# vimalabs/VIMA

Hardware: NVIDIA H100
Metric: policy steps/sec (batched action decode) (higher is better)
Workload: dtype f16 hi*hi + e4m3 cross terms (2 tensor pass-equivalents), f16 3-term in attention, fp32 accumulate/softmax/LN

## Files before the change

### vima_b200/build.py

```python
from __future__ import annotations

import hashlib
import os
import subprocess
import sys
from concurrent.futures import ThreadPoolExecutor

HERE = os.path.dirname(os.path.abspath(__file__))
CSRC = os.path.join(HERE, "csrc")
OUT_DIR = os.path.join(HERE, "_lib")
LIB_PATH = os.path.join(OUT_DIR, "libvima_b200.so")
SOURCES = ["api.cu", "gemm_tc_f16.cu", "gemm_tc_f16x3.cu", "gemm_tc_f16f8.cu", "gemm_tc_bf16.cu", "gemm_tc_bf16x3.cu", "gemm_wide_f16f8.cu", "norm.cu", "attention.cu", "attention_tc.cu", "attention_tc_paged.cu", "attention_tail.cu", "gemm_simt.cu", "misc.cu", "prepare.cu", "slots.cu"]
HEADERS = ["common.cuh", "kernels.h", "attention_tc.cuh", "gemm_tc.cuh", "gemm_tc_variants.cuh", "gemm_wide.cuh", os.path.join("..", "..", "include", "vima_b200.h")]
NVCC_FLAGS = [
    "-gencode", "arch=compute_90a,code=sm_90a", "-O3", "-lineinfo", "-std=c++17", "--expt-relaxed-constexpr",
    "-Xcompiler", "-fPIC", "-Xcompiler", "-fvisibility=hidden",
]


def _nvcc() -> str:
    for p in (os.environ.get("NVCC"), "/usr/local/cuda/bin/nvcc", "nvcc"):
        if p and (os.path.isfile(p) or p == "nvcc"):
            return p
    raise RuntimeError("nvcc not found")


def _digest() -> str:
    h = hashlib.sha256()
    for f in SOURCES + HEADERS:
        with open(os.path.join(CSRC, f), "rb") as fh:
            h.update(fh.read())
    h.update(" ".join(NVCC_FLAGS).encode())
    return h.hexdigest()


# ... 34 lines not shown
```

### vima_b200/csrc/api.cu

```cuda
#include <cstdarg>
#include <cstddef>
#include <cstdio>
#include <cstring>
#include <cstdlib>

#include "../../include/vima_b200.h"
#include "gemm_wide.cuh"
#include "kernels.h"

using namespace vima;
static_assert(VIMA_KV_PAGE_TOKENS == KV_PAGE_TOKENS, "page size of the C ABI and of the kernels");

struct vima_ctx {
  int device;
  int sm_count;
  int max_smem_optin;
  long long launches;
  char err[512];
  void* encode_tiled;
  int attn_tc;
  int attn_tail;
  int epi_prefetch;
  int attn_bias_tc;
  int gemm_wide;
};

struct DeviceGuard {
  int prev = -1;
  bool armed = false;
  cudaError_t enter(int dev) {
    cudaError_t e = cudaGetDevice(&prev);
    if (e != cudaSuccess) return e;
    if (prev == dev) return cudaSuccess;
    armed = true;
    return cudaSetDevice(dev);
  }
  ~DeviceGuard() {
    if (armed) cudaSetDevice(prev);
  }
};

static int fail(vima_ctx* c, int code, const char* fmt, ...) {
  if (c) {
    va_list ap;
    va_start(ap, fmt);
    vsnprintf(c->err, sizeof(c->err), fmt, ap);
    va_end(ap);
// ... 30 lines not shown
    return VIMA_OK;                                      \
  }

extern "C" {

int vima_abi_version(void) { return VIMA_B200_ABI_VERSION; }

int vima_set_option(vima_ctx* c, const char* key, const char* value) {
  if (!c) return VIMA_E_INVALID;
  if (!key || !value) return fail(c, VIMA_E_INVALID, "set_option: null key or value");
  if (!strcmp(key, "attn")) {
    if (!strcmp(value, "tc")) { c->attn_tc = 1; return VIMA_OK; }
    if (!strcmp(value, "mma")) { c->attn_tc = 0; return VIMA_OK; }
  } else if (!strcmp(key, "attn_tail")) {
    if (!strcmp(value, "kernel")) { c->attn_tail = 1; return VIMA_OK; }
    if (!strcmp(value, "off")) { c->attn_tail = 0; return VIMA_OK; }
  } else if (!strcmp(key, "attn_bias")) {
    if (!strcmp(value, "auto")) { c->attn_bias_tc = 0; return VIMA_OK; }
    if (!strcmp(value, "tc")) { c->attn_bias_tc = 1; return VIMA_OK; }
  } else if (!strcmp(key, "epi_prefetch")) {
    if (!strcmp(value, "0") || !strcmp(value, "1")) { c->epi_prefetch = value[0] == '1'; return VIMA_OK; }
  } else if (!strcmp(key, "gemm_wide")) {
    if (!strcmp(value, "0") || !strcmp(value, "1")) { c->gemm_wide = value[0] == '1'; return VIMA_OK; }
  }
  return fail(c, VIMA_E_INVALID, "set_option: unknown option %s=%s", key, value);
}

int vima_create(vima_ctx** out, int device) {
  if (!out) return VIMA_E_INVALID;
  *out = nullptr;
  int n = 0;
  if (cudaGetDeviceCount(&n) != cudaSuccess || device < 0 || device >= n) return VIMA_E_CUDA;
  cudaDeviceProp prop;
  if (cudaGetDeviceProperties(&prop, device) != cudaSuccess) return VIMA_E_CUDA;
  if (prop.major != 9 || prop.minor != 0) return VIMA_E_UNSUPPORTED;
  vima_ctx* c = new vima_ctx();
  memset(c, 0, sizeof(*c));
  c->device = device;
  c->sm_count = prop.multiProcessorCount;
  c->max_smem_optin = (int)prop.sharedMemPerBlockOptin;
  DeviceGuard guard;
  if (guard.enter(device) != cudaSuccess) { delete c; return VIMA_E_CUDA; }
  cudaFree(0);
  cudaDriverEntryPointQueryResult q;
  void* fn = nullptr;
  if (cudaGetDriverEntryPoint("cuTensorMapEncodeTiled", &fn, cudaEnableDefault, &q) != cudaSuccess || fn == nullptr) {
    delete c;
    return VIMA_E_CUDA;
  }
  c->encode_tiled = fn;
  c->attn_tc = 1; c->attn_tail = 1; c->epi_prefetch = 0; c->attn_bias_tc = 0; c->gemm_wide = 1;
  if (const char* e = getenv("VIMA_B200_ATTN")) vima_set_option(c, "attn", e);
  if (const char* e = getenv("VIMA_B200_ATTN_TAIL")) vima_set_option(c, "attn_tail", e);
  if (const char* e = getenv("VIMA_B200_EPI_PREFETCH")) vima_set_option(c, "epi_prefetch", e);
  if (const char* e = getenv("VIMA_B200_ATTN_BIAS")) vima_set_option(c, "attn_bias", e);
  if (const char* e = getenv("VIMA_B200_GEMM_WIDE")) vima_set_option(c, "gemm_wide", e);
  c->err[0] = 0;
  *out = c;
  return VIMA_OK;
}

void vima_destroy(vima_ctx* c) { delete c; }
const char* vima_last_error(vima_ctx* c) { return c ? c->err : "null context"; }
int vima_sm_count(vima_ctx* c) { return c ? c->sm_count : 0; }
int vima_sizeof_gemm_desc(void) { return (int)sizeof(vima_gemm_desc); }
int vima_sizeof_norm_desc(void) { return (int)sizeof(vima_norm_desc); }
int vima_sizeof_attn_desc(void) { return (int)sizeof(vima_attn_desc); }
int vima_sizeof_f32_gemm_group(void) { return (int)sizeof(vima_f32_gemm_group); }
int64_t vima_launch_count(vima_ctx* c) { return c ? c->launches : 0; }

int vima_split_f32(vima_ctx* c, const float* x, int64_t rows, int cols, int ldx, void* hi, void* lo, int ld16, int pad_cols, float scale,
                   int dtype, void* stream) {
  CHECK_CTX(c);
  if (!x || !hi || pad_cols < cols || pad_cols > ld16) return fail(c, VIMA_E_INVALID, "split_f32: bad arguments");
  LAUNCHED(c, launch_split(x, rows, cols, ldx, (unsigned short*)hi, (unsigned short*)lo, ld16, pad_cols, scale, dtype, (cudaStream_t)stream),
           "split_f32");
}

int vima_pack_weight(vima_ctx* c, const float* w, int n, int k, int transposed, int ldw, void* hi, void* lo, int ld16, float scale, int dtype,
// ... 220 lines not shown
  p.key_mask = d->key_mask; p.rel_bias = d->rel_bias;
  p.o_hi = (unsigned short*)d->o_hi; p.o_lo = (unsigned short*)d->o_lo; p.ldo = d->ldo;
  p.B = d->B; p.H = d->H; p.Lq = d->Lq; p.Lk = d->Lk; p.D = d->D;
  p.scale = d->scale; p.causal = d->causal; p.split = split; p.dtype = d->dtype;
  p.o_lo8 = (unsigned char*)d->o_lo8; p.o_hi8 = (unsigned char*)d->o_hi8; p.ldo8 = d->ldo8;
  p.kv_batch_rows = d->kv_batch_rows; p.mask_ld = d->mask_ld; p.q_pos0 = d->q_pos0; p.q_batch_rows = 0;
  p.q_pos = d->q_pos;
  p.kv_pages = d->kv_pages; p.kv_page_ld = d->kv_page_ld; p.kv_pool_pages = d->kv_pool_pages;
  p.kv_len = d->kv_len;
  if (d->kv_pages && ((d->causal && !d->q_pos) || d->rel_bias || d->kv_page_ld < 1 || d->kv_pool_pages < 1 ||
                      d->Lk > (long long)d->kv_page_ld * VIMA_KV_PAGE_TOKENS || (long long)d->kv_pool_pages * VIMA_KV_PAGE_TOKENS > 0x7fffffffll))
    return fail(c, VIMA_E_INVALID, "attention: paged k / v need q_pos (or non-causal attention), no relative bias, Lk <= kv_page_ld*%d (Lk %d, "
                "kv_page_ld %d) and 1 <= kv_pool_pages with kv_pool_pages*%d rows inside the 32-bit row range (kv_pool_pages %d)",
                VIMA_KV_PAGE_TOKENS, d->Lk, d->kv_page_ld, VIMA_KV_PAGE_TOKENS, d->kv_pool_pages);
  if (d->kv_len && (d->causal || d->q_pos || d->rel_bias))
    return fail(c, VIMA_E_INVALID, "attention: per-batch kv_len needs non-causal attention without q_pos or relative bias");
  if ((d->kv_batch_rows && d->kv_batch_rows < d->Lk) || (d->mask_ld && d->mask_ld < d->Lk) || d->q_pos0 < 0)
    return fail(c, VIMA_E_INVALID, "attention: kv_batch_rows / mask_ld must cover Lk, q_pos0 >= 0");
  if (d->q_pos && (!d->causal || d->rel_bias || d->Lq > d->Lk))
    return fail(c, VIMA_E_INVALID, "attention: per-batch q_pos needs causal attention, no relative bias and Lq <= Lk");
  if ((p.o_lo8 == nullptr) != (p.o_hi8 == nullptr) || (p.o_lo8 && ((p.ldo8 & 1) || d->dtype != DT_F16)))
    return fail(c, VIMA_E_INVALID, "attention: o_lo8/o_hi8 come together (fp16 format, even ldo8)");
  if (c->attn_tc && attention_tc_supported(p)) {
    const int tail = p.Lq % 128;
    if (c->attn_tail && p.Lq > 128 && tail >= 1 && tail <= ATTN_TAIL_MAX_ROWS && p.Lk <= ATTN_TAIL_MAX_LK) {
      AttnParams body = p;
      body.Lq = p.Lq - tail;
      body.q_batch_rows = p.Lq;
      cudaError_t e_ = launch_attention_tc(body, c->encode_tiled, (cudaStream_t)stream);
      if (e_ != cudaSuccess) return cuda_fail(c, e_, "attention_tc");
      c->launches++;
      LAUNCHED(c, launch_attention_tail(p, p.Lq - tail, tail, (cudaStream_t)stream), "attention_tail");
    }
    LAUNCHED(c, launch_attention_tc(p, c->encode_tiled, (cudaStream_t)stream), "attention_tc");
  }
  if (c->attn_tc && attention_bias_tc_supported(p) && (c->attn_bias_tc || attention_smem_bytes(p) > (size_t)c->max_smem_optin))
    LAUNCHED(c, launch_attention_tc(p, c->encode_tiled, (cudaStream_t)stream), "attention_bias_tc");
  {
    const size_t need = attention_smem_bytes(p);
    if (need > (size_t)c->max_smem_optin)
      return fail(c, VIMA_E_UNSUPPORTED,
                  "attention: Lk = %d keys of head_dim %d (%s operands%s) need %zu bytes of shared memory, the device offers %d: the "
                  "resident-K/V kernel takes Lk <= %d at this head_dim", d->Lk, d->D, split ? "split" : "single", d->rel_bias ? ", relative bias" : "",
                  need, c->max_smem_optin, attention_max_lk(p, (size_t)c->max_smem_optin));
  }
  LAUNCHED(c, launch_attention(p, (cudaStream_t)stream), "attention");
}

int vima_latent_attention(vima_ctx* c, const float* q, int ldq, int64_t q_batch_stride, const float* k, int ldk, const float* v, int ldv, float* o,
                          int ldo, int64_t N, int Lq, int Lk, int H, int d, float scale, void* stream) {
  CHECK_CTX(c);
  if (!q || !k || !v || !o) return fail(c, VIMA_E_INVALID, "latent_attention: null pointer");
  if (Lk < 1 || Lk > 16 || d < 1 || d > 128 || Lq < 0 || N < 0 || H < 1)
    return fail(c, VIMA_E_UNSUPPORTED, "latent_attention: 1..16 keys, head_dim <= 128 (Lk %d, d %d)", Lk, d);
  LatentAttnParams p;
  p.q = q; p.ldq = ldq; p.q_batch_stride = q_batch_stride; p.k = k; p.ldk = ldk; p.v = v; p.ldv = ldv; p.o = o; p.ldo = ldo;
  p.N = N; p.Lq = Lq; p.Lk = Lk; p.H = H; p.d = d; p.scale = scale;
// ... 296 lines not shown
```

### vima_b200/csrc/attention_tc.cu

```cuda
#include "attention_tc.cuh"

namespace vima {

namespace {

template <int DT>
__global__ void __launch_bounds__(ATC_THREADS, 2) attention_tc_kernel(const __grid_constant__ AttnTcParams P) {
  attention_tc_body<DT, 32, true, false, false>(P);
}
template <int DT, bool SPLIT>
__global__ void __launch_bounds__(ATC_THREADS, 2) attention_bias_tc_kernel(const __grid_constant__ AttnTcParams P) {
  attention_tc_body<DT, 64, SPLIT, true, false>(P);
}

bool aligned_operands(const AttnParams& p) {
  auto al = [](const void* q) { return ((uintptr_t)q & 15) == 0; };
  return al(p.q_hi) && al(p.q_lo) && al(p.k_hi) && al(p.k_lo) && al(p.v_hi) && al(p.v_lo) && al(p.o_hi) && al(p.o_lo) && al(p.o_lo8) &&
         al(p.o_hi8);
}

}

long long attention_kv_rows(const AttnParams& p) {
  if (p.kv_pages) return (long long)p.kv_pool_pages * KV_PAGE_TOKENS;
  return (long long)p.B * (p.kv_batch_rows ? p.kv_batch_rows : p.Lk);
}

bool attention_tc_supported(const AttnParams& p) {
  const int qbr = p.q_batch_rows ? p.q_batch_rows : p.Lq;
  if (!aligned_operands(p)) return false;
  return p.D == 32 && p.split != 0 && p.rel_bias == nullptr && p.q_lo && p.k_lo && p.v_lo && (p.ldq % 8 == 0) && (p.ldk % 8 == 0) &&
         (p.ldv % 8 == 0) && (p.ldo % 8 == 0) && (p.o_lo8 == nullptr || p.ldo8 % 8 == 0) && p.H <= 65535 && p.B <= 65535 && p.Lk >= 1 &&
         attention_kv_rows(p) <= 0x7fffffffll && (long long)p.B * qbr <= 0x7fffffffll;
}

bool attention_bias_tc_supported(const AttnParams& p) {
  if (!aligned_operands(p)) return false;
  const bool split_ok = p.split ? (p.q_lo && p.k_lo && p.v_lo) : (!p.q_lo && !p.k_lo && !p.v_lo);
  return p.D == 64 && p.rel_bias != nullptr && !p.causal && p.q_pos == nullptr && p.q_pos0 == 0 && p.q_batch_rows == 0 && p.Lq == p.Lk &&
         (p.kv_batch_rows == 0 || p.kv_batch_rows == p.Lk) && (p.mask_ld == 0 || p.mask_ld == p.Lk) && split_ok && (p.ldq % 8 == 0) &&
         (p.ldk % 8 == 0) && (p.ldv % 8 == 0) && (p.ldo % 2 == 0) && (p.o_lo8 == nullptr || p.ldo8 % 2 == 0) && p.H <= 65535 &&
         p.B <= 65535 && p.Lk >= 1 && (long long)p.B * p.Lk <= 0x7fffffffll;
}

cudaError_t launch_attention_tc(const AttnParams& p, void* encode_fn, cudaStream_t stream) {
  if (p.B == 0 || p.Lq == 0) return cudaSuccess;
  const bool bias = p.rel_bias != nullptr;
  const int D = bias ? 64 : 32;
  AttnTcParams P;
  memset(&P, 0, sizeof(P));
  P.a = p;
  const long long kv_rows = attention_kv_rows(p);
  const long long q_rows = (long long)p.B * (p.q_batch_rows ? p.q_batch_rows : p.Lq);
  auto map = [&](CUtensorMap* tm, const void* base, long long rows, int ld, int box_rows) {
    return encode_tmap_2d(encode_fn, tm, p.dtype == DT_BF16 ? CU_TENSOR_MAP_DATA_TYPE_BFLOAT16 : CU_TENSOR_MAP_DATA_TYPE_FLOAT16, base,
                          (uint64_t)rows, (uint64_t)p.H * D, (uint64_t)ld * 2, (uint32_t)D, (uint32_t)box_rows,
                          D == 32 ? CU_TENSOR_MAP_SWIZZLE_64B : CU_TENSOR_MAP_SWIZZLE_128B, CU_TENSOR_MAP_L2_PROMOTION_L2_128B) == CUDA_SUCCESS;
  };
  bool ok = map(&P.tm_q_hi, p.q_hi, q_rows, p.ldq, ATC_BM) && map(&P.tm_k_hi, p.k_hi, kv_rows, p.ldk, ATC_KC);
  if (p.split) ok = ok && map(&P.tm_q_lo, p.q_lo, q_rows, p.ldq, ATC_BM) && map(&P.tm_k_lo, p.k_lo, kv_rows, p.ldk, ATC_KC);
  if (!ok) return cudaErrorInvalidValue;
  dim3 grid((p.Lq + ATC_BM - 1) / ATC_BM, p.H, p.B);
  const bool bf = p.dtype == DT_BF16;
  if (!bias && p.kv_pages) return launch_attention_tc_paged(P, grid, stream);
  if (!bias) return bf ? launch_t<attention_tc_kernel<DT_BF16>, 32, false>(P, grid, stream) : launch_t<attention_tc_kernel<DT_F16>, 32, false>(P, grid, stream);
  if (bf) return p.split ? launch_t<attention_bias_tc_kernel<DT_BF16, true>, 64, true>(P, grid, stream)
                         : launch_t<attention_bias_tc_kernel<DT_BF16, false>, 64, true>(P, grid, stream);
  return p.split ? launch_t<attention_bias_tc_kernel<DT_F16, true>, 64, true>(P, grid, stream)
                 : launch_t<attention_bias_tc_kernel<DT_F16, false>, 64, true>(P, grid, stream);
}

}
```

### vima_b200/csrc/attention_tc.cuh

```cuda
#pragma once
#include "kernels.h"

namespace vima {

struct AttnTcParams {
  AttnParams a;
  CUtensorMap tm_q_hi, tm_q_lo, tm_k_hi, tm_k_lo;
};
cudaError_t launch_attention_tc_paged(const AttnTcParams& P, dim3 grid, cudaStream_t stream);

namespace {

constexpr int ATC_THREADS = 256;
constexpr int ATC_BM = 128, ATC_KC = 64;
constexpr int ATC_WIN = ATC_BM + ATC_KC - 1;

template <int D, bool BIAS>
struct AtcSmem {
  static constexpr int Q_PART = ATC_BM * D * 2;
  static constexpr int K_PART = ATC_KC * D * 2;
  static constexpr int QH = 0, QL = Q_PART;
  static constexpr int K = 2 * Q_PART;
  static constexpr int VT = K + 4 * K_PART;
  static constexpr int MASK = VT + 4 * K_PART;
  static constexpr int BIAS_W = MASK + 2 * ATC_KC * 4;
  static constexpr int BAR = BIAS_W + (BIAS ? 2 * 192 * 4 : 0);
  static constexpr int BYTES = BAR + 32;
};

template <int DT, int D, bool SPLIT, bool BIAS, bool PAGED>
__device__ __forceinline__ void attention_tc_body(const AttnTcParams& P) {
  using S = AtcSmem<D, BIAS>;
  constexpr int PARTS = SPLIT ? 2 : 1;
  constexpr int VN = D / 4;
  const AttnParams& p = P.a;
  extern __shared__ __align__(1024) uint8_t sm[];
  float* maskadd = reinterpret_cast<float*>(sm + S::MASK);
  float* sbias = reinterpret_cast<float*>(sm + S::BIAS_W);
  uint64_t* bars = reinterpret_cast<uint64_t*>(sm + S::BAR);
  uint64_t* q_full = bars + 0;
  uint64_t* k_full = bars + 1;

  const int tid = threadIdx.x, warp = tid >> 5, lane = tid & 31;
  const int wg = warp >> 2;
  const int q0 = blockIdx.x * ATC_BM, h = blockIdx.y, b = blockIdx.z;
  const int Lq = p.Lq;
  const int mld = !BIAS && p.mask_ld ? p.mask_ld : p.Lk;
  const int qbr = !BIAS && p.q_batch_rows ? p.q_batch_rows : Lq;
  int qp0 = 0, Lk = p.Lk;
  if constexpr (!BIAS) attn_batch_keys(p, b, qbr, qp0, Lk);
  const uint32_t sbase = smem_u32(sm);
// ... 57 lines not shown
  const float c_l2 = p.scale * LOG2E;
  auto desc_qk = [](uint32_t addr) { return D == 32 ? wgmma_desc_sw64(addr) : wgmma_desc_sw128(addr); };
  const uint64_t dqh = desc_qk(sbase + S::QH + wg * (S::Q_PART / 2)), dql = desc_qk(sbase + S::QL + wg * (S::Q_PART / 2));
  const int vj = tid >> 2, vd = tid & 3;
  uint32_t k_use[2] = {0u, 0u};
  float o[D / 2], m_run[2], l_run[2];
  int n = n_plan;
  for (int pass = 0; pass < 2; ++pass) {
#pragma unroll
    for (int i = 0; i < D / 2; ++i) o[i] = 0.f;
    m_run[0] = m_run[1] = -INFINITY;
    l_run[0] = l_run[1] = 0.f;
    if (tid == 0) {
      load_k(0, 0);
      if (n > 1) load_k(1, 1);
    }
    if (pass == 0) mbar_wait(q_full, 0);
    for (int c = 0; c < n; ++c) {
      const int stage = c & 1;
      const int k0 = c * ATC_KC;
      mbar_wait(&k_full[stage], k_use[stage] & 1u);
      k_use[stage]++;
      float s[32];
      {
        const uint32_t k_addr = sbase + S::K + stage * 2 * S::K_PART;
        const uint64_t dkh = desc_qk(k_addr), dkl = desc_qk(k_addr + S::K_PART);
        wgmma_fence();
#pragma unroll
        for (int k = 0; k < D / 16; ++k) wgmma_m64nNk16_ss<DT, 64>(s, dqh + 2 * k, dkh + 2 * k, (uint32_t)(k != 0));
        if constexpr (SPLIT) {
#pragma unroll
          for (int k = 0; k < D / 16; ++k) wgmma_m64nNk16_ss<DT, 64>(s, dql + 2 * k, dkh + 2 * k, 1u);
#pragma unroll
          for (int k = 0; k < D / 16; ++k) wgmma_m64nNk16_ss<DT, 64>(s, dqh + 2 * k, dkl + 2 * k, 1u);
        }
        wgmma_commit();
      }
      {
        uint4 vh[VN / 8], vl[VN / 8];
#pragma unroll
        for (int i = 0; i < VN / 8; ++i) vh[i] = vl[i] = make_uint4(0u, 0u, 0u, 0u);
        if (k0 + vj < Lk) {
          const size_t off = (size_t)(chunk_row(c) + vj) * p.ldv + x_col + vd * VN;
#pragma unroll
          for (int i = 0; i < VN / 8; ++i) {
            vh[i] = __ldg(reinterpret_cast<const uint4*>(p.v_hi + off + 8 * i));
            if constexpr (SPLIT) vl[i] = __ldg(reinterpret_cast<const uint4*>(p.v_lo + off + 8 * i));
          }
        }
        if (c + 1 < n) stage_chunk(c + 1);
        uint8_t* vt = sm + S::VT + stage * 2 * S::K_PART;
        uint32_t wh[VN / 2], wl[VN / 2];
#pragma unroll
        for (int i = 0; i < VN / 8; ++i) {
          wh[4 * i] = vh[i].x; wh[4 * i + 1] = vh[i].y; wh[4 * i + 2] = vh[i].z; wh[4 * i + 3] = vh[i].w;
          wl[4 * i] = vl[i].x; wl[4 * i + 1] = vl[i].y; wl[4 * i + 2] = vl[i].z; wl[4 * i + 3] = vl[i].w;
        }
#pragma unroll
        for (int e = 0; e < VN; ++e) {
          const int nn = vd * VN + e;
          const int off = nn * 128 + ((((vj >> 3) ^ (nn & 7))) << 4) + (vj & 7) * 2;
          *reinterpret_cast<unsigned short*>(vt + off) = (unsigned short)(wh[e >> 1] >> (16 * (e & 1)));
          if constexpr (SPLIT) *reinterpret_cast<unsigned short*>(vt + S::K_PART + off) = (unsigned short)(wl[e >> 1] >> (16 * (e & 1)));
        }
        fence_proxy_async();
      }
      wgmma_wait<0>();
      wgmma_fence_acc(s);
      const float* mk = maskadd + stage * ATC_KC;
      const float* bw = sbias + stage * 192 + (ATC_BM - 1) - r_loc;
      float mx[2] = {-INFINITY, -INFINITY};
#pragma unroll
      for (int g = 0; g < 8; ++g)
#pragma unroll
        for (int e = 0; e < 4; ++e) {
          const int jj = 8 * g + 2 * qd + (e & 1), key = k0 + jj;
          const float mm = mk[jj];
          float y;
          if constexpr (BIAS) {
            y = s[4 * g + e] * c_l2;
            y += bw[jj - 8 * (e >> 1)];
            y += mm;
          } else {
            y = fmaf(s[4 * g + e], c_l2, mm);
            if (p.causal && key > q0 + r_loc + 8 * (e >> 1) + qp0) y = CAUSAL_L2 + mm;
          }
          s[4 * g + e] = y;
          mx[e >> 1] = fmaxf(mx[e >> 1], y);
        }
      float f[2];
#pragma unroll
      for (int hh = 0; hh < 2; ++hh) {
        mx[hh] = fmaxf(mx[hh], __shfl_xor_sync(0xffffffffu, mx[hh], 1));
        mx[hh] = fmaxf(mx[hh], __shfl_xor_sync(0xffffffffu, mx[hh], 2));
        const float m_new = fmaxf(m_run[hh], mx[hh]);
        f[hh] = ex2_approx(m_run[hh] - m_new);
        m_run[hh] = m_new;
      }
      uint32_t ph[16], pl[16];
      float ps[2] = {0.f, 0.f};
#pragma unroll
      for (int i = 0; i < 16; ++i) {
        const int hh = i & 1;
        const float p0 = ex2_approx(s[2 * i] - m_run[hh]), p1 = ex2_approx(s[2 * i + 1] - m_run[hh]);
        ps[hh] += p0 + p1;
        split2<DT>(p0, p1, ph[i], pl[i]);
      }
#pragma unroll
      for (int hh = 0; hh < 2; ++hh) l_run[hh] = l_run[hh] * f[hh] + ps[hh];
#pragma unroll
      for (int i = 0; i < D / 2; ++i) o[i] *= f[(i >> 1) & 1];
      named_bar_sync(1, ATC_THREADS);
      if (tid == 0 && c + 2 < n) load_k(c + 2, stage);
      {
        const uint32_t vt_addr = sbase + S::VT + stage * 2 * S::K_PART;
        const uint64_t dvh = wgmma_desc_sw128(vt_addr), dvl = wgmma_desc_sw128(vt_addr + S::K_PART);
        wgmma_fence();
#pragma unroll
        for (int kk = 0; kk < ATC_KC / 16; ++kk) {
          const uint32_t ah[4] = {ph[4 * kk], ph[4 * kk + 1], ph[4 * kk + 2], ph[4 * kk + 3]};
          const uint32_t al[4] = {pl[4 * kk], pl[4 * kk + 1], pl[4 * kk + 2], pl[4 * kk + 3]};
          wgmma_m64nNk16_rs<DT, D>(o, ah, dvh + 2 * kk, 1u);
          if constexpr (SPLIT) {
            wgmma_m64nNk16_rs<DT, D>(o, al, dvh + 2 * kk, 1u);
            wgmma_m64nNk16_rs<DT, D>(o, ah, dvl + 2 * kk, 1u);
          }
        }
        wgmma_commit();
        wgmma_wait<0>();
        wgmma_fence_acc(o);
      }
    }
    if (pass == 1 || !may_rerun) break;
    if constexpr (!BIAS) {
      const int undone = (r_loc < rows_here && !(m_run[0] > EXIT_L2)) || (r_loc + 8 < rows_here && !(m_run[1] > EXIT_L2));
      if (!__syncthreads_or(undone)) break;
      n = n_all;
      stage_chunk(0);
      __syncthreads();
    }
  }
#pragma unroll
  for (int hh = 0; hh < 2; ++hh) {
    float l = l_run[hh];
    l += __shfl_xor_sync(0xffffffffu, l, 1);
    l += __shfl_xor_sync(0xffffffffu, l, 2);
    const int row = q0 + r_loc + 8 * hh;
    if (row < Lq) {
      const float inv = 1.0f / l;
      const size_t brow = (size_t)b * qbr + row;
#pragma unroll
      for (int g = 0; g < D / 8; ++g) attn_store_pair<DT>(p, brow, x_col + 8 * g + 2 * qd, o[4 * g + 2 * hh] * inv, o[4 * g + 2 * hh + 1] * inv);
    }
  }
}

template <auto KERNEL, int D, bool BIAS>
cudaError_t launch_t(const AttnTcParams& P, dim3 grid, cudaStream_t stream) {
  constexpr int smem = AtcSmem<D, BIAS>::BYTES;
  const cudaError_t e = raise_smem_ceiling<KERNEL>(smem);
  if (e != cudaSuccess) return e;
  KERNEL<<<grid, ATC_THREADS, smem, stream>>>(P);
  return cudaGetLastError();
}

}

}
```

### vima_b200/csrc/kernels.h

```cpp
#pragma once
#include "common.cuh"

namespace vima {

struct NormParams {
  const float* x; long long rows; int cols; int ldx;
  const float* add; int ld_add;
  const float* w; const float* b;
  float eps; int rms;
  const float* w2; const float* b2; float eps2;
  float* out_f32; int ld_o32;
  float* out2_f32; int ld_o2;
  unsigned short* out_hi; unsigned short* out_lo; int ld_o16;
  int dtype;
  unsigned char* out_lo8; unsigned char* out_hi8; int ld_o8;
  float* stats_out; float stats_eps;
};
cudaError_t launch_norm(const NormParams& p, cudaStream_t stream);
cudaError_t launch_row_stats_finalize(const float* partial, long long rows, int parts, int cols, float eps, int rms, float* stats,
                                      cudaStream_t stream);

struct AttnParams {
  const unsigned short *q_hi, *q_lo; int ldq;
  const unsigned short *k_hi, *k_lo; int ldk;
// ... 44 lines not shown
  split2<DT>(x0, x1, hi, lo);
  const size_t off = brow * p.ldo + col;
  *reinterpret_cast<uint32_t*>(p.o_hi + off) = hi;
  if (p.o_lo) *reinterpret_cast<uint32_t*>(p.o_lo + off) = lo;
  if (p.o_lo8) {
    const float2 f = __half22float2(*reinterpret_cast<const __half2*>(&hi));
    const size_t off8 = brow * p.ldo8 + col;
    unsigned short l8, h8;
    asm("cvt.rn.satfinite.e4m3x2.f32 %0, %1, %2;" : "=h"(l8) : "f"((x1 - f.y) * F8_ACT_LO_SCALE), "f"((x0 - f.x) * F8_ACT_LO_SCALE));
    asm("cvt.rn.satfinite.e4m3x2.f32 %0, %1, %2;" : "=h"(h8) : "f"(x1 * F8_ACT_HI_SCALE), "f"(x0 * F8_ACT_HI_SCALE));
    *reinterpret_cast<unsigned short*>(p.o_lo8 + off8) = l8;
    *reinterpret_cast<unsigned short*>(p.o_hi8 + off8) = h8;
  }
}
constexpr int ATTN_TAIL_MAX_ROWS = 8;
constexpr int ATTN_TAIL_MAX_LK = 512;
cudaError_t launch_attention(const AttnParams& p, cudaStream_t stream);
size_t attention_smem_bytes(const AttnParams& p);
int attention_max_lk(const AttnParams& p, size_t smem_limit);
long long attention_kv_rows(const AttnParams& p);
bool attention_tc_supported(const AttnParams& p);
bool attention_bias_tc_supported(const AttnParams& p);
cudaError_t launch_attention_tc(const AttnParams& p, void* encode_tiled_fn, cudaStream_t stream);
cudaError_t launch_attention_tail(const AttnParams& p, int row0, int nt, cudaStream_t stream);

struct SmallAttnParams {
  const float* qkv; int ld;
  unsigned short *o_hi, *o_lo; int ldo; float* o_f32;
  long long N; int S, H, W; float scale; int dtype;
};
cudaError_t launch_small_attention(const SmallAttnParams& p, cudaStream_t stream);

struct LatentAttnParams {
  const float* q; int ldq; long long q_batch_stride;
  const float* k; int ldk;
  const float* v; int ldv;
  float* o; int ldo;
  long long N; int Lq, Lk, H, d; float scale;
};
cudaError_t launch_latent_attention(const LatentAttnParams& p, cudaStream_t stream);

struct SimtGemmGroup {
  const float* x; int ldx;
  const float* w; int ldw;
  const float* b;
  float* y; int ldy;
// ... 80 lines not shown
```

Baseline: 1633.

## Add resident-KV attention kernel that keeps all keys/values in shared memory per head

Adds an attention kernel that launches one CTA per (head, batch), loads the whole K and transposed V for short sequences (up to 320 keys) into shared memory once, then has its two warpgroups pull 64-row query blocks through a shared atomic counter with double-buffered Q loads. The target cost is the repeated K/V staging and per-chunk barriers that the tiled kernel pays for every 128-row query tile. The shared QK/softmax/PV pieces are factored into helpers that both kernels use. The new path is on by default when shapes fit, and it trades grid parallelism for reuse, so small batch×head counts may leave SMs idle.

New measurement: 1650, median of 6. +1.0%, better.

```diff
diff --git a/vima_b200/build.py b/vima_b200/build.py
--- a/vima_b200/build.py
+++ b/vima_b200/build.py
@@ -10,7 +10,7 @@
 CSRC = os.path.join(HERE, "csrc")
 OUT_DIR = os.path.join(HERE, "_lib")
 LIB_PATH = os.path.join(OUT_DIR, "libvima_b200.so")
-SOURCES = ["api.cu", "gemm_tc_f16.cu", "gemm_tc_f16x3.cu", "gemm_tc_f16f8.cu", "gemm_tc_bf16.cu", "gemm_tc_bf16x3.cu", "gemm_wide_f16f8.cu", "norm.cu", "attention.cu", "attention_tc.cu", "attention_tc_paged.cu", "attention_tail.cu", "gemm_simt.cu", "misc.cu", "prepare.cu", "slots.cu"]
+SOURCES = ["api.cu", "gemm_tc_f16.cu", "gemm_tc_f16x3.cu", "gemm_tc_f16f8.cu", "gemm_tc_bf16.cu", "gemm_tc_bf16x3.cu", "gemm_wide_f16f8.cu", "norm.cu", "attention.cu", "attention_tc.cu", "attention_tc_paged.cu", "attention_resident.cu", "attention_tail.cu", "gemm_simt.cu", "misc.cu", "prepare.cu", "slots.cu"]
 HEADERS = ["common.cuh", "kernels.h", "attention_tc.cuh", "gemm_tc.cuh", "gemm_tc_variants.cuh", "gemm_wide.cuh", os.path.join("..", "..", "include", "vima_b200.h")]
 NVCC_FLAGS = [
     "-gencode", "arch=compute_90a,code=sm_90a", "-O3", "-lineinfo", "-std=c++17", "--expt-relaxed-constexpr",
diff --git a/vima_b200/csrc/api.cu b/vima_b200/csrc/api.cu
--- a/vima_b200/csrc/api.cu
+++ b/vima_b200/csrc/api.cu
@@ -23,6 +23,7 @@
   int epi_prefetch;
   int attn_bias_tc;
   int gemm_wide;
+  int attn_resident;
 };
 
 struct DeviceGuard {
@@ -99,6 +100,8 @@
     if (!strcmp(value, "0") || !strcmp(value, "1")) { c->epi_prefetch = value[0] == '1'; return VIMA_OK; }
   } else if (!strcmp(key, "gemm_wide")) {
     if (!strcmp(value, "0") || !strcmp(value, "1")) { c->gemm_wide = value[0] == '1'; return VIMA_OK; }
+  } else if (!strcmp(key, "attn_resident")) {
+    if (!strcmp(value, "0") || !strcmp(value, "1")) { c->attn_resident = value[0] == '1'; return VIMA_OK; }
   }
   return fail(c, VIMA_E_INVALID, "set_option: unknown option %s=%s", key, value);
 }
@@ -126,12 +129,13 @@
     return VIMA_E_CUDA;
   }
   c->encode_tiled = fn;
-  c->attn_tc = 1; c->attn_tail = 1; c->epi_prefetch = 0; c->attn_bias_tc = 0; c->gemm_wide = 1;
+  c->attn_tc = 1; c->attn_tail = 1; c->epi_prefetch = 0; c->attn_bias_tc = 0; c->gemm_wide = 1; c->attn_resident = 1;
   if (const char* e = getenv("VIMA_B200_ATTN")) vima_set_option(c, "attn", e);
   if (const char* e = getenv("VIMA_B200_ATTN_TAIL")) vima_set_option(c, "attn_tail", e);
   if (const char* e = getenv("VIMA_B200_EPI_PREFETCH")) vima_set_option(c, "epi_prefetch", e);
   if (const char* e = getenv("VIMA_B200_ATTN_BIAS")) vima_set_option(c, "attn_bias", e);
   if (const char* e = getenv("VIMA_B200_GEMM_WIDE")) vima_set_option(c, "gemm_wide", e);
+  if (const char* e = getenv("VIMA_B200_ATTN_RESIDENT")) vima_set_option(c, "attn_resident", e);
   c->err[0] = 0;
   *out = c;
   return VIMA_OK;
@@ -398,17 +402,22 @@
   if ((p.o_lo8 == nullptr) != (p.o_hi8 == nullptr) || (p.o_lo8 && ((p.ldo8 & 1) || d->dtype != DT_F16)))
     return fail(c, VIMA_E_INVALID, "attention: o_lo8/o_hi8 come together (fp16 format, even ldo8)");
   if (c->attn_tc && attention_tc_supported(p)) {
+    const bool resident = c->attn_resident && attention_resident_supported(p);
+    auto launch_body = [&](const AttnParams& q) {
+      return resident ? launch_attention_resident(q, c->encode_tiled, (cudaStream_t)stream) : launch_attention_tc(q, c->encode_tiled, (cudaStream_t)stream);
+    };
+    const char* body_name = resident ? "attention_resident" : "attention_tc";
     const int tail = p.Lq % 128;
     if (c->attn_tail && p.Lq > 128 && tail >= 1 && tail <= ATTN_TAIL_MAX_ROWS && p.Lk <= ATTN_TAIL_MAX_LK) {
       AttnParams body = p;
       body.Lq = p.Lq - tail;
       body.q_batch_rows = p.Lq;
-      cudaError_t e_ = launch_attention_tc(body, c->encode_tiled, (cudaStream_t)stream);
-      if (e_ != cudaSuccess) return cuda_fail(c, e_, "attention_tc");
+      cudaError_t e_ = launch_body(body);
+      if (e_ != cudaSuccess) return cuda_fail(c, e_, body_name);
       c->launches++;
       LAUNCHED(c, launch_attention_tail(p, p.Lq - tail, tail, (cudaStream_t)stream), "attention_tail");
     }
-    LAUNCHED(c, launch_attention_tc(p, c->encode_tiled, (cudaStream_t)stream), "attention_tc");
+    LAUNCHED(c, launch_body(p), body_name);
   }
   if (c->attn_tc && attention_bias_tc_supported(p) && (c->attn_bias_tc || attention_smem_bytes(p) > (size_t)c->max_smem_optin))
     LAUNCHED(c, launch_attention_tc(p, c->encode_tiled, (cudaStream_t)stream), "attention_bias_tc");
diff --git a/vima_b200/csrc/attention_resident.cu b/vima_b200/csrc/attention_resident.cu
--- /dev/null
+++ b/vima_b200/csrc/attention_resident.cu
@@ -0,0 +1,35 @@
+#include "attention_tc.cuh"
+
+namespace vima {
+
+bool attention_resident_supported(const AttnParams& p) {
+  return attention_tc_supported(p) && p.kv_pages == nullptr && p.Lk <= ATTN_RESIDENT_MAX_LK && p.Lq <= ATTN_RESIDENT_MAX_LK;
+}
+
+namespace {
+
+template <int DT>
+__global__ void __launch_bounds__(ATC_THREADS, 2) attention_resident_kernel(const __grid_constant__ AttnTcParams P) {
+  attention_resident_body<DT>(P);
+}
+
+template <int DT>
+cudaError_t launch_resident_t(const AttnTcParams& P, cudaStream_t stream) {
+  const cudaError_t e = raise_smem_ceiling<attention_resident_kernel<DT>>(ArSmem::BYTES);
+  if (e != cudaSuccess) return e;
+  attention_resident_kernel<DT><<<dim3(1, P.a.H, P.a.B), ATC_THREADS, ArSmem::BYTES, stream>>>(P);
+  return cudaGetLastError();
+}
+
+}
+
+cudaError_t launch_attention_resident(const AttnParams& p, void* encode_fn, cudaStream_t stream) {
+  if (p.B == 0 || p.Lq == 0) return cudaSuccess;
+  AttnTcParams P;
+  memset(&P, 0, sizeof(P));
+  P.a = p;
+  if (!encode_attention_tc_maps(P, encode_fn, ATC_KC)) return cudaErrorInvalidValue;
+  return p.dtype == DT_BF16 ? launch_resident_t<DT_BF16>(P, stream) : launch_resident_t<DT_F16>(P, stream);
+}
+
+}
diff --git a/vima_b200/csrc/attention_tc.cu b/vima_b200/csrc/attention_tc.cu
--- a/vima_b200/csrc/attention_tc.cu
+++ b/vima_b200/csrc/attention_tc.cu
@@ -43,13 +43,9 @@
          p.B <= 65535 && p.Lk >= 1 && (long long)p.B * p.Lk <= 0x7fffffffll;
 }
 
-cudaError_t launch_attention_tc(const AttnParams& p, void* encode_fn, cudaStream_t stream) {
-  if (p.B == 0 || p.Lq == 0) return cudaSuccess;
-  const bool bias = p.rel_bias != nullptr;
-  const int D = bias ? 64 : 32;
-  AttnTcParams P;
-  memset(&P, 0, sizeof(P));
-  P.a = p;
+bool encode_attention_tc_maps(AttnTcParams& P, void* encode_fn, int q_box) {
+  const AttnParams& p = P.a;
+  const int D = p.rel_bias ? 64 : 32;
   const long long kv_rows = attention_kv_rows(p);
   const long long q_rows = (long long)p.B * (p.q_batch_rows ? p.q_batch_rows : p.Lq);
   auto map = [&](CUtensorMap* tm, const void* base, long long rows, int ld, int box_rows) {
@@ -57,9 +53,18 @@
                           (uint64_t)rows, (uint64_t)p.H * D, (uint64_t)ld * 2, (uint32_t)D, (uint32_t)box_rows,
                           D == 32 ? CU_TENSOR_MAP_SWIZZLE_64B : CU_TENSOR_MAP_SWIZZLE_128B, CU_TENSOR_MAP_L2_PROMOTION_L2_128B) == CUDA_SUCCESS;
   };
-  bool ok = map(&P.tm_q_hi, p.q_hi, q_rows, p.ldq, ATC_BM) && map(&P.tm_k_hi, p.k_hi, kv_rows, p.ldk, ATC_KC);
-  if (p.split) ok = ok && map(&P.tm_q_lo, p.q_lo, q_rows, p.ldq, ATC_BM) && map(&P.tm_k_lo, p.k_lo, kv_rows, p.ldk, ATC_KC);
-  if (!ok) return cudaErrorInvalidValue;
+  bool ok = map(&P.tm_q_hi, p.q_hi, q_rows, p.ldq, q_box) && map(&P.tm_k_hi, p.k_hi, kv_rows, p.ldk, ATC_KC);
+  if (p.split) ok = ok && map(&P.tm_q_lo, p.q_lo, q_rows, p.ldq, q_box) && map(&P.tm_k_lo, p.k_lo, kv_rows, p.ldk, ATC_KC);
+  return ok;
+}
+
+cudaError_t launch_attention_tc(const AttnParams& p, void* encode_fn, cudaStream_t stream) {
+  if (p.B == 0 || p.Lq == 0) return cudaSuccess;
+  const bool bias = p.rel_bias != nullptr;
+  AttnTcParams P;
+  memset(&P, 0, sizeof(P));
+  P.a = p;
+  if (!encode_attention_tc_maps(P, encode_fn, ATC_BM)) return cudaErrorInvalidValue;
   dim3 grid((p.Lq + ATC_BM - 1) / ATC_BM, p.H, p.B);
   const bool bf = p.dtype == DT_BF16;
   if (!bias && p.kv_pages) return launch_attention_tc_paged(P, grid, stream);
diff --git a/vima_b200/csrc/attention_tc.cuh b/vima_b200/csrc/attention_tc.cuh
--- a/vima_b200/csrc/attention_tc.cuh
+++ b/vima_b200/csrc/attention_tc.cuh
@@ -8,6 +8,7 @@
   CUtensorMap tm_q_hi, tm_q_lo, tm_k_hi, tm_k_lo;
 };
 cudaError_t launch_attention_tc_paged(const AttnTcParams& P, dim3 grid, cudaStream_t stream);
+bool encode_attention_tc_maps(AttnTcParams& P, void* encode_fn, int q_box);
 
 namespace {
 
@@ -27,6 +28,147 @@
   static constexpr int BAR = BIAS_W + (BIAS ? 2 * 192 * 4 : 0);
   static constexpr int BYTES = BAR + 32;
 };
+
+
+template <int DT, int D, bool SPLIT>
+__device__ __forceinline__ void atc_qk(float (&s)[32], uint64_t dqh, uint64_t dql, uint32_t k_addr) {
+  constexpr int PART = ATC_KC * D * 2;
+  auto desc_qk = [](uint32_t addr) { return D == 32 ? wgmma_desc_sw64(addr) : wgmma_desc_sw128(addr); };
+  const uint64_t dkh = desc_qk(k_addr), dkl = desc_qk(k_addr + PART);
+  wgmma_fence();
+#pragma unroll
+  for (int k = 0; k < D / 16; ++k) wgmma_m64nNk16_ss<DT, 64>(s, dqh + 2 * k, dkh + 2 * k, (uint32_t)(k != 0));
+  if constexpr (SPLIT) {
+#pragma unroll
+    for (int k = 0; k < D / 16; ++k) wgmma_m64nNk16_ss<DT, 64>(s, dql + 2 * k, dkh + 2 * k, 1u);
+#pragma unroll
+    for (int k = 0; k < D / 16; ++k) wgmma_m64nNk16_ss<DT, 64>(s, dqh + 2 * k, dkl + 2 * k, 1u);
+  }
+  wgmma_commit();
+}
+
+template <int D>
+struct AtcVShare {
+  uint4 h[D / 32], l[D / 32];
+};
+template <int D, bool SPLIT>
+__device__ __forceinline__ AtcVShare<D> atc_v_load(const AttnParams& p, bool valid, size_t off) {
+  AtcVShare<D> v;
+#pragma unroll
+  for (int i = 0; i < D / 32; ++i) v.h[i] = v.l[i] = make_uint4(0u, 0u, 0u, 0u);
+  if (valid) {
+#pragma unroll
+    for (int i = 0; i < D / 32; ++i) {
+      v.h[i] = __ldg(reinterpret_cast<const uint4*>(p.v_hi + off + 8 * i));
+      if constexpr (SPLIT) v.l[i] = __ldg(reinterpret_cast<const uint4*>(p.v_lo + off + 8 * i));
+    }
+  }
+  return v;
+}
+template <int D, bool SPLIT>
+__device__ __forceinline__ void atc_v_store(uint8_t* vt, const AtcVShare<D>& v, int vj, int vd) {
+  constexpr int VN = D / 4, PART = ATC_KC * D * 2;
+  uint32_t wh[VN / 2], wl[VN / 2];
+#pragma unroll
+  for (int i = 0; i < VN / 8; ++i) {
+    wh[4 * i] = v.h[i].x; wh[4 * i + 1] = v.h[i].y; wh[4 * i + 2] = v.h[i].z; wh[4 * i + 3] = v.h[i].w;
+    wl[4 * i] = v.l[i].x; wl[4 * i + 1] = v.l[i].y; wl[4 * i + 2] = v.l[i].z; wl[4 * i + 3] = v.l[i].w;
+  }
+#pragma unroll
+  for (int e = 0; e < VN; ++e) {
+    const int nn = vd * VN + e;
+    const int off = nn * 128 + ((((vj >> 3) ^ (nn & 7))) << 4) + (vj & 7) * 2;
+    *reinterpret_cast<unsigned short*>(vt + off) = (unsigned short)(wh[e >> 1] >> (16 * (e & 1)));
+    if constexpr (SPLIT) *reinterpret_cast<unsigned short*>(vt + PART + off) = (unsigned short)(wl[e >> 1] >> (16 * (e & 1)));
+  }
+}
+
+template <int DT, int D, bool BIAS>
+__device__ __forceinline__ void atc_softmax(float (&s)[32], const float* mk, const float* bw, float c_l2, bool causal, int k0, int qrow,
+                                            int qd, float (&m_run)[2], float (&l_run)[2], float (&o)[D / 2], uint32_t (&ph)[16],
+                                            uint32_t (&pl)[16]) {
+  float mx[2] = {-INFINITY, -INFINITY};
+#pragma unroll
+  for (int g = 0; g < 8; ++g)
+#pragma unroll
+    for (int e = 0; e < 4; ++e) {
+      const int jj = 8 * g + 2 * qd + (e & 1), key = k0 + jj;
+      const float mm = mk[jj];
+      float y;
+      if constexpr (BIAS) {
+        y = s[4 * g + e] * c_l2;
+        y += bw[jj - 8 * (e >> 1)];
+        y += mm;
+      } else {
+        y = fmaf(s[4 * g + e], c_l2, mm);
+        if (causal && key > qrow + 8 * (e >> 1)) y = CAUSAL_L2 + mm;
+      }
+      s[4 * g + e] = y;
+      mx[e >> 1] = fmaxf(mx[e >> 1], y);
+    }
+  float f[2];
+#pragma unroll
+  for (int hh = 0; hh < 2; ++hh) {
+    mx[hh] = fmaxf(mx[hh], __shfl_xor_sync(0xffffffffu, mx[hh], 1));
+    mx[hh] = fmaxf(mx[hh], __shfl_xor_sync(0xffffffffu, mx[hh], 2));
+    const float m_new = fmaxf(m_run[hh], mx[hh]);
+    f[hh] = ex2_approx(m_run[hh] - m_new);
+    m_run[hh] = m_new;
+  }
+  float ps[2] = {0.f, 0.f};
+#pragma unroll
+  for (int i = 0; i < 16; ++i) {
+    const int hh = i & 1;
+    const float p0 = ex2_approx(s[2 * i] - m_run[hh]), p1 = ex2_approx(s[2 * i + 1] - m_run[hh]);
+    ps[hh] += p0 + p1;
+    split2<DT>(p0, p1, ph[i], pl[i]);
+  }
+#pragma unroll
+  for (int hh = 0; hh < 2; ++hh) l_run[hh] = l_run[hh] * f[hh] + ps[hh];
+#pragma unroll
+  for (int i = 0; i < D / 2; ++i) o[i] *= f[(i >> 1) & 1];
+}
+
+template <int DT, int D, bool SPLIT>
+__device__ __forceinline__ void atc_pv(float (&o)[D / 2], const uint32_t (&ph)[16], const uint32_t (&pl)[16], uint32_t vt_addr) {
+  constexpr int PART = ATC_KC * D * 2;
+  const uint64_t dvh = wgmma_desc_sw128(vt_addr), dvl = wgmma_desc_sw128(vt_addr + PART);
+  wgmma_fence();
+#pragma unroll
+  for (int kk = 0; kk < ATC_KC / 16; ++kk) {
+    const uint32_t ah[4] = {ph[4 * kk], ph[4 * kk + 1], ph[4 * kk + 2], ph[4 * kk + 3]};
+    const uint32_t al[4] = {pl[4 * kk], pl[4 * kk + 1], pl[4 * kk + 2], pl[4 * kk + 3]};
+    wgmma_m64nNk16_rs<DT, D>(o, ah, dvh + 2 * kk, 1u);
+    if constexpr (SPLIT) {
+      wgmma_m64nNk16_rs<DT, D>(o, al, dvh + 2 * kk, 1u);
+      wgmma_m64nNk16_rs<DT, D>(o, ah, dvl + 2 * kk, 1u);
+    }
+  }
+  wgmma_commit();
+  wgmma_wait<0>();
+  wgmma_fence_acc(o);
+}
+
+__device__ __forceinline__ bool atc_undone(const float (&m_run)[2], int r, int rows) {
+  return (r < rows && !(m_run[0] > EXIT_L2)) || (r + 8 < rows && !(m_run[1] > EXIT_L2));
+}
+
+template <int DT, int D>
+__device__ __forceinline__ void atc_store(const AttnParams& p, const float (&o)[D / 2], const float (&l_run)[2], size_t brow0, int row,
+                                          int Lq, int x_col, int qd) {
+#pragma unroll
+  for (int hh = 0; hh < 2; ++hh) {
+    float l = l_run[hh];
+    l += __shfl_xor_sync(0xffffffffu, l, 1);
+    l += __shfl_xor_sync(0xffffffffu, l, 2);
+    if (row + 8 * hh < Lq) {
+      const float inv = 1.0f / l;
+      const size_t brow = brow0 + row + 8 * hh;
+#pragma unroll
+      for (int g = 0; g < D / 8; ++g) attn_store_pair<DT>(p, brow, x_col + 8 * g + 2 * qd, o[4 * g + 2 * hh] * inv, o[4 * g + 2 * hh + 1] * inv);
+    }
+  }
+}
 
 template <int DT, int D, bool SPLIT, bool BIAS, bool PAGED>
 __device__ __forceinline__ void attention_tc_body(const AttnTcParams& P) {
@@ -130,136 +272,166 @@
       mbar_wait(&k_full[stage], k_use[stage] & 1u);
       k_use[stage]++;
       float s[32];
+      atc_qk<DT, D, SPLIT>(s, dqh, dql, sbase + S::K + stage * 2 * S::K_PART);
       {
-        const uint32_t k_addr = sbase + S::K + stage * 2 * S::K_PART;
-        const uint64_t dkh = desc_qk(k_addr), dkl = desc_qk(k_addr + S::K_PART);
-        wgmma_fence();
-#pragma unroll
-        for (int k = 0; k < D / 16; ++k) wgmma_m64nNk16_ss<DT, 64>(s, dqh + 2 * k, dkh + 2 * k, (uint32_t)(k != 0));
-        if constexpr (SPLIT) {
-#pragma unroll
-          for (int k = 0; k < D / 16; ++k) wgmma_m64nNk16_ss<DT, 64>(s, dql + 2 * k, dkh + 2 * k, 1u);
-#pragma unroll
-          for (int k = 0; k < D / 16; ++k) wgmma_m64nNk16_ss<DT, 64>(s, dqh + 2 * k, dkl + 2 * k, 1u);
-        }
-        wgmma_commit();
-      }
-      {
-        uint4 vh[VN / 8], vl[VN / 8];
-#pragma unroll
-        for (int i = 0; i < VN / 8; ++i) vh[i] = vl[i] = make_uint4(0u, 0u, 0u, 0u);
-        if (k0 + vj < Lk) {
-          const size_t off = (size_t)(chunk_row(c) + vj) * p.ldv + x_col + vd * VN;
-#pragma unroll
-          for (int i = 0; i < VN / 8; ++i) {
-            vh[i] = __ldg(reinterpret_cast<const uint4*>(p.v_hi + off + 8 * i));
-            if constexpr (SPLIT) vl[i] = __ldg(reinterpret_cast<const uint4*>(p.v_lo + off + 8 * i));
-          }
-        }
+        const AtcVShare<D> v = atc_v_load<D, SPLIT>(p, k0 + vj < Lk, (size_t)(chunk_row(c) + vj) * p.ldv + x_col + vd * VN);
         if (c + 1 < n) stage_chunk(c + 1);
-        uint8_t* vt = sm + S::VT + stage * 2 * S::K_PART;
-        uint32_t wh[VN / 2], wl[VN / 2];
-#pragma unroll
-        for (int i = 0; i < VN / 8; ++i) {
-          wh[4 * i] = vh[i].x; wh[4 * i + 1] = vh[i].y; wh[4 * i + 2] = vh[i].z; wh[4 * i + 3] = vh[i].w;
-          wl[4 * i] = vl[i].x; wl[4 * i + 1] = vl[i].y; wl[4 * i + 2] = vl[i].z; wl[4 * i + 3] = vl[i].w;
-        }
-#pragma unroll
-        for (int e = 0; e < VN; ++e) {
-          const int nn = vd * VN + e;
-          const int off = nn * 128 + ((((vj >> 3) ^ (nn & 7))) << 4) + (vj & 7) * 2;
-          *reinterpret_cast<unsigned short*>(vt + off) = (unsigned short)(wh[e >> 1] >> (16 * (e & 1)));
-          if constexpr (SPLIT) *reinterpret_cast<unsigned short*>(vt + S::K_PART + off) = (unsigned short)(wl[e >> 1] >> (16 * (e & 1)));
-        }
+        atc_v_store<D, SPLIT>(sm + S::VT + stage * 2 * S::K_PART, v, vj, vd);
         fence_proxy_async();
       }
       wgmma_wait<0>();
       wgmma_fence_acc(s);
-      const float* mk = maskadd + stage * ATC_KC;
-      const float* bw = sbias + stage * 192 + (ATC_BM - 1) - r_loc;
-      float mx[2] = {-INFINITY, -INFINITY};
-#pragma unroll
-      for (int g = 0; g < 8; ++g)
-#pragma unroll
-        for (int e = 0; e < 4; ++e) {
-          const int jj = 8 * g + 2 * qd + (e & 1), key = k0 + jj;
-          const float mm = mk[jj];
-          float y;
-          if constexpr (BIAS) {
-            y = s[4 * g + e] * c_l2;
-            y += bw[jj - 8 * (e >> 1)];
-            y += mm;
-          } else {
-            y = fmaf(s[4 * g + e], c_l2, mm);
-            if (p.causal && key > q0 + r_loc + 8 * (e >> 1) + qp0) y = CAUSAL_L2 + mm;
-          }
-          s[4 * g + e] = y;
-          mx[e >> 1] = fmaxf(mx[e >> 1], y);
-        }
-      float f[2];
-#pragma unroll
-      for (int hh = 0; hh < 2; ++hh) {
-        mx[hh] = fmaxf(mx[hh], __shfl_xor_sync(0xffffffffu, mx[hh], 1));
-        mx[hh] = fmaxf(mx[hh], __shfl_xor_sync(0xffffffffu, mx[hh], 2));
-        const float m_new = fmaxf(m_run[hh], mx[hh]);
-        f[hh] = ex2_approx(m_run[hh] - m_new);
-        m_run[hh] = m_new;
-      }
       uint32_t ph[16], pl[16];
-      float ps[2] = {0.f, 0.f};
-#pragma unroll
-      for (int i = 0; i < 16; ++i) {
-        const int hh = i & 1;
-        const float p0 = ex2_approx(s[2 * i] - m_run[hh]), p1 = ex2_approx(s[2 * i + 1] - m_run[hh]);
-        ps[hh] += p0 + p1;
-        split2<DT>(p0, p1, ph[i], pl[i]);
-      }
-#pragma unroll
-      for (int hh = 0; hh < 2; ++hh) l_run[hh] = l_run[hh] * f[hh] + ps[hh];
-#pragma unroll
-      for (int i = 0; i < D / 2; ++i) o[i] *= f[(i >> 1) & 1];
+      atc_softmax<DT, D, BIAS>(s, maskadd + stage * ATC_KC, sbias + stage * 192 + (ATC_BM - 1) - r_loc, c_l2, p.causal, k0,
+                               q0 + r_loc + qp0, qd, m_run, l_run, o, ph, pl);
       named_bar_sync(1, ATC_THREADS);
       if (tid == 0 && c + 2 < n) load_k(c + 2, stage);
-      {
-        const uint32_t vt_addr = sbase + S::VT + stage * 2 * S::K_PART;
-        const uint64_t dvh = wgmma_desc_sw128(vt_addr), dvl = wgmma_desc_sw128(vt_addr + S::K_PART);
-        wgmma_fence();
-#pragma unroll
-        for (int kk = 0; kk < ATC_KC / 16; ++kk) {
-          const uint32_t ah[4] = {ph[4 * kk], ph[4 * kk + 1], ph[4 * kk + 2], ph[4 * kk + 3]};
-          const uint32_t al[4] = {pl[4 * kk], pl[4 * kk + 1], pl[4 * kk + 2], pl[4 * kk + 3]};
-          wgmma_m64nNk16_rs<DT, D>(o, ah, dvh + 2 * kk, 1u);
-          if constexpr (SPLIT) {
-            wgmma_m64nNk16_rs<DT, D>(o, al, dvh + 2 * kk, 1u);
-            wgmma_m64nNk16_rs<DT, D>(o, ah, dvl + 2 * kk, 1u);
-          }
-        }
-        wgmma_commit();
-        wgmma_wait<0>();
-        wgmma_fence_acc(o);
-      }
+      atc_pv<DT, D, SPLIT>(o, ph, pl, sbase + S::VT + stage * 2 * S::K_PART);
     }
     if (pass == 1 || !may_rerun) break;
     if constexpr (!BIAS) {
-      const int undone = (r_loc < rows_here && !(m_run[0] > EXIT_L2)) || (r_loc + 8 < rows_here && !(m_run[1] > EXIT_L2));
-      if (!__syncthreads_or(undone)) break;
+      if (!__syncthreads_or(atc_undone(m_run, r_loc, rows_here))) break;
       n = n_all;
       stage_chunk(0);
       __syncthreads();
     }
   }
-#pragma unroll
-  for (int hh = 0; hh < 2; ++hh) {
-    float l = l_run[hh];
-    l += __shfl_xor_sync(0xffffffffu, l, 1);
-    l += __shfl_xor_sync(0xffffffffu, l, 2);
-    const int row = q0 + r_loc + 8 * hh;
-    if (row < Lq) {
-      const float inv = 1.0f / l;
-      const size_t brow = (size_t)b * qbr + row;
-#pragma unroll
-      for (int g = 0; g < D / 8; ++g) attn_store_pair<DT>(p, brow, x_col + 8 * g + 2 * qd, o[4 * g + 2 * hh] * inv, o[4 * g + 2 * hh + 1] * inv);
-    }
+  atc_store<DT, D>(p, o, l_run, (size_t)b * qbr, q0 + r_loc, Lq, x_col, qd);
+}
+
+struct ArSmem {
+  static constexpr int CHUNKS = ATTN_RESIDENT_MAX_LK / ATC_KC;
+  static constexpr int PART = ATC_KC * 32 * 2;
+  static constexpr int K = 0;
+  static constexpr int VT = K + CHUNKS * 2 * PART;
+  static constexpr int Q = VT + CHUNKS * 2 * PART;
+  static constexpr int MASK = Q + 2 * 2 * PART;
+  static constexpr int BAR = MASK + CHUNKS * ATC_KC * 4;
+  static constexpr int BYTES = BAR + 3 * 8 + 3 * 4;
+};
+static_assert(ATTN_RESIDENT_MAX_LK % ATC_KC == 0, "the resident key cap is a whole number of chunks");
+
+__device__ __forceinline__ bool named_bar_or(int id, int n, bool pred) {
+  uint32_t r;
+  asm volatile("{\n\t.reg .pred p, q;\n\tsetp.ne.u32 p, %1, 0;\n\tbar.red.or.pred q, %2, %3, p;\n\tselp.u32 %0, 1, 0, q;\n\t}"
+               : "=r"(r) : "r"((uint32_t)pred), "r"(id), "r"(n) : "memory");
+  return r != 0u;
+}
+
+template <int DT>
+__device__ __forceinline__ void attention_resident_body(const AttnTcParams& P) {
+  using S = ArSmem;
+  constexpr int D = 32;
+  const AttnParams& p = P.a;
+  extern __shared__ __align__(1024) uint8_t sm[];
+  float* maskadd = reinterpret_cast<float*>(sm + S::MASK);
+  uint64_t* bars = reinterpret_cast<uint64_t*>(sm + S::BAR);
+  uint64_t* kv_full = bars + 0;
+  uint64_t* q_full = bars + 1;
+  int* next = reinterpret_cast<int*>(bars + 3);
+
+  const int tid = threadIdx.x, warp = tid >> 5, lane = tid & 31;
+  const int wg = warp >> 2;
+  const int h = blockIdx.y, b = blockIdx.z;
+  const int Lq = p.Lq;
+  const int mld = p.mask_ld ? p.mask_ld : p.Lk;
+  const int qbr = p.q_batch_rows ? p.q_batch_rows : Lq;
+  int qp0 = 0, Lk = p.Lk;
+  attn_batch_keys(p, b, qbr, qp0, Lk);
+  const uint32_t sbase = smem_u32(sm);
+  const int n_all = (Lk + ATC_KC - 1) / ATC_KC;
+  const int n_blocks = (Lq + ATC_KC - 1) / ATC_KC;
+  if ((sbase & 1023u) != 0u) {
+    if (tid == 0) printf("vima_b200: attention_resident shared memory window is not 1024-byte aligned\n");
+    __trap();
+  }
+  const int x_col = h * D;
+  const int kv_row0 = (int)attn_kv_row<false>(p, b, 0);
+  if (tid == 0) {
+    mbar_init(kv_full, 1);
+    mbar_init(&q_full[0], 1);
+    mbar_init(&q_full[1], 1);
+    next[0] = 2;
+    fence_barrier_init();
+    tma_prefetch_desc(&P.tm_q_hi);
+    tma_prefetch_desc(&P.tm_q_lo);
+    tma_prefetch_desc(&P.tm_k_hi);
+    tma_prefetch_desc(&P.tm_k_lo);
+  }
+  for (int j = tid; j < n_all * ATC_KC; j += ATC_THREADS) maskadd[j] = attn_key_mask_term(p, b, mld, j, Lk);
+  __syncthreads();
+
+  auto load_q = [&](int i, int w) {
+    uint8_t* dst = sm + S::Q + w * 2 * S::PART;
+    const int row = b * qbr + (n_blocks - 1 - i) * ATC_KC;
+    mbar_arrive_expect_tx(&q_full[w], (uint32_t)(2 * S::PART));
+    tma_load_2d(dst, &P.tm_q_hi, &q_full[w], x_col, row);
+    tma_load_2d(dst + S::PART, &P.tm_q_lo, &q_full[w], x_col, row);
+  };
+  if (tid == 0) {
+    mbar_arrive_expect_tx(kv_full, (uint32_t)(n_all * 2 * S::PART));
+    for (int c = 0; c < n_all; ++c) {
+      uint8_t* dst = sm + S::K + c * 2 * S::PART;
+      tma_load_2d(dst, &P.tm_k_hi, kv_full, x_col, kv_row0 + c * ATC_KC);
+      tma_load_2d(dst + S::PART, &P.tm_k_lo, kv_full, x_col, kv_row0 + c * ATC_KC);
+    }
+    load_q(0, 0);
+    if (n_blocks > 1) load_q(1, 1);
+  }
+  {
+    const int vj = tid >> 2, vd = tid & 3;
+    AtcVShare<D> v[S::CHUNKS];
+#pragma unroll
+    for (int c = 0; c < S::CHUNKS; ++c)
+      v[c] = atc_v_load<D, true>(p, c < n_all && c * ATC_KC + vj < Lk, (size_t)(kv_row0 + c * ATC_KC + vj) * p.ldv + x_col + vd * (D / 4));
+#pragma unroll
+    for (int c = 0; c < S::CHUNKS; ++c)
+      if (c < n_all) atc_v_store<D, true>(sm + S::VT + c * 2 * S::PART, v[c], vj, vd);
+    fence_proxy_async();
+  }
+  __syncthreads();
+  mbar_wait(kv_full, 0);
+
+  const int r_w = (warp & 3) * 16 + (lane >> 2);
+  const int qd = lane & 3;
+  const float c_l2 = p.scale * LOG2E;
+  const uint64_t dqh = wgmma_desc_sw64(sbase + S::Q + wg * 2 * S::PART), dql = wgmma_desc_sw64(sbase + S::Q + wg * 2 * S::PART + S::PART);
+  auto wg_bar_or = [&](bool pred) { return wg == 0 ? named_bar_or(2, 128, pred) : named_bar_or(3, 128, pred); };
+  uint32_t q_use = 0u;
+  for (int i = wg; i < n_blocks;) {
+    const int q0 = (n_blocks - 1 - i) * ATC_KC;
+    const int rows_here = min(ATC_KC, Lq - q0);
+    int n = n_all;
+    if (p.causal) n = min(Lk - 1, q0 + rows_here - 1 + qp0) / ATC_KC + 1;
+    const bool may_rerun = p.causal && n < n_all;
+    mbar_wait(&q_full[wg], q_use & 1u);
+    q_use++;
+    float o[D / 2], m_run[2], l_run[2];
+    for (int pass = 0; pass < 2; ++pass) {
+#pragma unroll
+      for (int k = 0; k < D / 2; ++k) o[k] = 0.f;
+      m_run[0] = m_run[1] = -INFINITY;
+      l_run[0] = l_run[1] = 0.f;
+      for (int c = 0; c < n; ++c) {
+        float s[32];
+        atc_qk<DT, D, true>(s, dqh, dql, sbase + S::K + c * 2 * S::PART);
+        wgmma_wait<0>();
+        wgmma_fence_acc(s);
+        uint32_t ph[16], pl[16];
+        atc_softmax<DT, D, false>(s, maskadd + c * ATC_KC, nullptr, c_l2, p.causal, c * ATC_KC, q0 + r_w + qp0, qd, m_run, l_run, o, ph, pl);
+        atc_pv<DT, D, true>(o, ph, pl, sbase + S::VT + c * 2 * S::PART);
+      }
+      if (!wg_bar_or(pass == 0 && may_rerun && atc_undone(m_run, r_w, rows_here))) break;
+      n = n_all;
+    }
+    if ((tid & 127) == 0) {
+      const int nx = atomicAdd(&next[0], 1);
+      next[1 + wg] = nx;
+      if (nx < n_blocks) load_q(nx, wg);
+    }
+    atc_store<DT, D>(p, o, l_run, (size_t)b * qbr, q0 + r_w, Lq, x_col, qd);
+    wg_bar_or(false);
+    i = next[1 + wg];
   }
 }
 
diff --git a/vima_b200/csrc/kernels.h b/vima_b200/csrc/kernels.h
--- a/vima_b200/csrc/kernels.h
+++ b/vima_b200/csrc/kernels.h
@@ -90,6 +90,9 @@
 bool attention_tc_supported(const AttnParams& p);
 bool attention_bias_tc_supported(const AttnParams& p);
 cudaError_t launch_attention_tc(const AttnParams& p, void* encode_tiled_fn, cudaStream_t stream);
+constexpr int ATTN_RESIDENT_MAX_LK = 320;
+bool attention_resident_supported(const AttnParams& p);
+cudaError_t launch_attention_resident(const AttnParams& p, void* encode_tiled_fn, cudaStream_t stream);
 cudaError_t launch_attention_tail(const AttnParams& p, int row0, int nt, cudaStream_t stream);
 
 struct SmallAttnParams {
```
